# LeeBY68/Hier-SLAM

Measured on AMD Instinct MI355X. Metric: fwd+bwd renders/sec @1200x680, 500k Gaussians, 4-level tree; grad max-abs-err vs ref, higher is better.
Workload: dtype f32; 1 GPU; semantic fwd+bwd render, 1200x680, P=500000 slam Gaussians, K=26 semantic channels, dense upstream grads on colour/semantic/depth/median/opacity; P=500000, visible=480888, num_rendered=1136056, width=1200, height=680, K=26, parallelism=single GPU, keyframes_per_rank=1

## Files before the change

### hier-slam_amd/csrc/hsr_render_bwd_q.hip

```cpp
#include "hsr_bwd_tile.h"

#ifdef HSR_TRACE
#define HSR_TRACE_SLOTS 8
__device__ unsigned long long g_hsr_trace_q[16384 * HSR_TRACE_SLOTS];
extern "C" int hsr_debug_read_trace_q(unsigned long long* host, int n)
{
    return (int)hipMemcpyFromSymbol(host, HIP_SYMBOL(g_hsr_trace_q), sizeof(unsigned long long) * (size_t)n);
}
#define TR_NOW() clock64()
#define TR_ADD(acc, t0) (acc) += (unsigned long long)(clock64() - (t0))
#else
#define TR_NOW() 0ll
#define TR_ADD(acc, t0) ((void)0)
#endif

namespace {

constexpr int Q_ROWS = 16;
constexpr int Q_CAP = 40;
constexpr int Q_SEG_DUMMY = Q_CAP;
constexpr int Q_SEG_ZERO = Q_CAP + 1;
constexpr int Q_NSEG = Q_CAP + 2;
constexpr int Q_SEGW = 17;
constexpr int Q_SEGB = Q_SEGW * 4;
constexpr int Q_PANEL = Q_NSEG * Q_SEGW;
constexpr int Q_ORD = 20;
constexpr int Q_TB = 36;
constexpr int Q_ENTB = 48;
static_assert(2 * Q_PANEL >= 64 * 17, "the two panels double as the prologue's transposition scratch");
static_assert(Q_ROWS * Q_TB <= Q_SEG_ZERO * Q_SEGW, "the emission table overlays the W panel below its zero segment");

template <int KC, int BATCH, bool GEO, bool CL = false, bool SEMA = false>
__global__ void __launch_bounds__(256, (SEMA || (!GEO && KC + 5 > 16)) ? 3 : 4) render_bwd_q_kernel(RenderBwdArgs a)
{
    static_assert(!SEMA || (GEO && KC % 4 == 0 && KC > 0), "the semantic -> alpha pass is a geometry-only pass over whole float4s of features");
    constexpr int ENTB = SEMA ? Q_ENTB + 4 * KC : Q_ENTB;
    constexpr int REC4 = ENTB / 16;
    constexpr int NCH = GEO ? 0 : KC + 5;
    constexpr int NG = GEO ? 0 : (NCH + 15) / 16;
    constexpr int NGA = NG > 0 ? NG : 1;
    static_assert(NG <= 2, "at most 32 direct channels per launch");
    static_assert(BATCH <= 256 && (BATCH + 1) * ENTB < 65536, "batch slots are bytes, record offsets 16 bits");
    __shared__ float4 s_ent[REC4 * (BATCH + 1)];
    __shared__ int s_id[BATCH];
    __shared__ uint16_t s_mask[BATCH + 2];
    __shared__ uint8_t s_list[4][256];
    __shared__ uint8_t s_lcnt[4][4];
    __shared__ uint8_t s_flat[4][256];
    __shared__ int s_wmax[4];
    __shared__ __attribute__((aligned(16))) float s_pan[4][2 * Q_PANEL];
    __shared__ uint2 s_ord[4][4][Q_ORD];
    __shared__ uint32_t s_rowent[4][Q_ROWS];
    __shared__ __attribute__((aligned(16))) uint32_t s_cid[4][Q_ROWS];
    __shared__ float s_medj[BATCH];
    __shared__ uint8_t s_segtab[4][Q_ROWS][4];

    const int tile = hsr_block_tile(blockIdx.x, hsr_num_tiles(a.W, a.H));
    if (tile >= hsr_num_tiles(a.W, a.H)) return;
    const int t = threadIdx.x, lane = t & 63, wv = t >> 6, gq = lane >> 4, l16 = lane & 15;
    const TileGeom tg = tile_geom_sub(tile, a.W, a.H, t);
    const bool inside = tg.inside;
    const size_t N = (size_t)a.W * a.H;
    const size_t pix_id = (size_t)a.W * tg.py + tg.px;
    float pfx = tg.pfx, pfy = tg.pfy;
    asm volatile("" : "+v"(pfx), "+v"(pfy));
    const uint2 range = a.ranges[tile];
    float* pw = s_pan[wv];
    float* pq = s_pan[wv] + Q_PANEL;
    unsigned long long tr_stage = 0, tr_loop = 0, tr_flush = 0, tr_iters = 0, tr_chunks = 0, tr_accepted = 0, tr_setup = 0;
    (void)tr_setup;
    const long long tr_t0 = TR_NOW();
    (void)tr_stage; (void)tr_loop; (void)tr_flush; (void)tr_iters; (void)tr_chunks; (void)tr_accepted; (void)tr_t0;

    if (t < REC4) s_ent[REC4 * BATCH + t] = make_float4(0.f, 0.f, 0.f, 0.f);

    const size_t pix_ld = inside ? pix_id : 0;
    const float inm = inside ? 1.f : 0.f;
    const float T_final_ld = a.final_T[pix_ld];
    const int last_contributor_ld = (int)a.n_contrib[pix_ld];
    const int median_at_ld = (int)a.median_pos[pix_ld];
    float dpx0 = a.dL_dpix[pix_ld], dpx1 = a.dL_dpix[N + pix_ld], dpx2 = a.dL_dpix[2 * N + pix_ld];
    float dpd = a.dL_dpix_depth[pix_ld], dpm = a.dL_dpix_median[pix_ld], dpo = a.dL_dpix_opacity[pix_ld];
    float semv[KC > 0 ? KC : 1];
#pragma unroll
    for (int c = 0; c < KC; c++) semv[c] = a.dL_dpix_sem[(size_t)min((SEMA ? a.sem_c0 : 0) + c, a.K - 1) * N + pix_ld];
    if (SEMA) {
#pragma unroll
        for (int c = 0; c < KC; c++) semv[c] = (a.sem_c0 + c < a.K) ? semv[c] * inm : 0.f;
        dpx0 = dpx1 = dpx2 = dpd = dpm = dpo = 0.f;
    }
    dpx0 *= inm; dpx1 *= inm; dpx2 *= inm; dpd *= inm; dpm *= inm; dpo *= inm;
    const float T_final = T_final_ld * inm;
    float T = T_final;
    const int last_contributor = inside ? last_contributor_ld : 0;
    const int median_at = (inside ? median_at_ld : 0) - 1;

    int wmax = last_contributor;
#pragma unroll
    for (int o = 32; o > 0; o >>= 1) wmax = max(wmax, __shfl_xor(wmax, o));
    if (lane == 0) s_wmax[wv] = wmax;

    float Breg[NGA][16];
    if (!GEO) {
        float gv[NGA][16];
#pragma unroll
        for (int g = 0; g < NG; g++)
#pragma unroll
            for (int c = 0; c < 16; c++) {
                const int ch = 16 * g + c;
                float v = 0.f;
                if (ch < KC) {
                    v = (ch < a.K) ? semv[ch < KC ? ch : 0] * inm : 0.f;
                } else if (ch == KC) v = dpx0;
                else if (ch == KC + 1) v = dpx1;
                else if (ch == KC + 2) v = dpx2;
                else if (ch == KC + 3) v = dpd;
                else if (ch == KC + 4) v = dpo;
                gv[g][c] = v;
            }
#pragma unroll
        for (int g = 0; g < NG; g++) {
            HSR_BWD_TRANSPOSE_B(pw, lane, gv[g], Breg[g]);
        }
    }
    if (lane < 2 * Q_SEGW) {
        if (GEO) pw[Q_SEG_ZERO * 2 * Q_SEGW + lane] = 0.f;
        else (lane < Q_SEGW ? pw : pq - Q_SEGW)[Q_SEG_ZERO * Q_SEGW + lane] = 0.f;
    }
    __syncthreads();
    const int hi_all = max(max(s_wmax[0], s_wmax[1]), max(s_wmax[2], s_wmax[3]));
    const long long tr_t1 = TR_NOW();
    (void)tr_t1;

    const float ntfbg = -T_final * (a.bg[0] * dpx0 + a.bg[1] * dpx1 + a.bg[2] * dpx2);
    const float kx2 = (a.W) / HSR_LOG2E, ky2 = (a.H) / HSR_LOG2E;
    float Racc = 0.f;
    char* const panb = reinterpret_cast<char*>(&s_pan[0][0]);
    const char* const entb = reinterpret_cast<const char*>(&s_ent[0]);
    constexpr uint32_t SEGB = GEO ? 2 * Q_SEGB : Q_SEGB;
    const uint32_t wave_off = (uint32_t)(wv * 2 * Q_PANEL * 4);
    const uint32_t lane16_off = wave_off + (uint32_t)(l16 * (GEO ? 8 : 4));
    const uint2 DUMMY_ELEM = make_uint2((uint32_t)(BATCH * ENTB), (uint32_t)Q_SEG_DUMMY * SEGB);
    uint2* const ordp = &s_ord[wv][gq][0];

    HSR_BWD_STAGING_DECLARE();
    HSR_BWD_STAGING_PRIME(hi_all, BATCH);

    auto flush = [&](int nrows) {
        wave_lds_fence();
        const uint32_t st = *reinterpret_cast<const uint32_t*>(&s_segtab[wv][l16][0]);
        const float cxg = pfx - (float)(l16 & 3) + 1.5f, cyg = pfy - (float)(l16 >> 2) + 1.5f;
        constexpr bool ALL_IN_LINE0 = CL && NCH <= 9;
        int colg[NGA], tslot[NGA];
#pragma unroll
        for (int g = 0; g < NGA; g++) {
            const int ch = 16 * g + l16;
            const int chl = ch < KC ? (ch < a.K ? ch : -1) : (ch < KC + 5 ? a.K + (ch - KC) : -1);
            const int col = (GEO || chl < 0) ? -1 : hsr_grow_col(CL ? 1 : 0, a.K, chl);
            colg[g] = (col >= 16 && !ALL_IN_LINE0) ? col : -1;
            tslot[g] = (CL && col >= 7 && col < 16) ? col - 7 : -1;
        }
        f32x4 acc[NGA];
#pragma unroll
        for (int g = 0; g < NGA; g++) acc[g] = f32x4{0.f, 0.f, 0.f, 0.f};
        if (!GEO) {
            float av[16];
#pragma unroll
            for (int g4 = 0; g4 < 4; g4++) {
                const float* sp = pw + ((st >> (8 * g4)) & 0xFFu) * Q_SEGW + gq;
#pragma unroll
                for (int i = 0; i < 4; i++) av[4 * g4 + i] = sp[4 * i];
            }
            asm volatile("" : "+v"(av[0]), "+v"(av[1]), "+v"(av[2]), "+v"(av[3]), "+v"(av[4]), "+v"(av[5]), "+v"(av[6]), "+v"(av[7]));
            asm volatile("" : "+v"(av[8]), "+v"(av[9]), "+v"(av[10]), "+v"(av[11]), "+v"(av[12]), "+v"(av[13]), "+v"(av[14]), "+v"(av[15]));
            if (NG == 1) {
                f32x4 acc2 = f32x4{0.f, 0.f, 0.f, 0.f};
#pragma unroll
                for (int m = 0; m < 16; m += 2) {
                    acc[0] = __builtin_amdgcn_mfma_f32_16x16x4f32(av[m], Breg[0][m], acc[0], 0, 0, 0);
                    acc2 = __builtin_amdgcn_mfma_f32_16x16x4f32(av[m + 1], Breg[0][m + 1], acc2, 0, 0, 0);
                }
                acc[0] += acc2;
            } else {
#pragma unroll
                for (int m = 0; m < 16; m++)
#pragma unroll
                    for (int g = 0; g < NG; g++)
                        acc[g] = __builtin_amdgcn_mfma_f32_16x16x4f32(av[m], Breg[g][m], acc[g], 0, 0, 0);
            }
        }
        float o[7];
        const uint32_t myseg = (st >> (8 * gq)) & 0xFFu;
        float qv[16], wd[GEO ? 16 : 1], medsum;
        if (GEO) {
            const float2* qp = reinterpret_cast<const float2*>(pw) + myseg * Q_SEGW;
#pragma unroll
            for (int i = 0; i < 16; i++) {
                const float2 v = qp[i];
                qv[i] = v.x;
                wd[GEO ? i : 0] = v.y;
            }
            medsum = 0.f;
        } else {
            const float* qp = pq + myseg * Q_SEGW;
#pragma unroll
            for (int i = 0; i < 16; i++) qv[i] = qp[i];
            medsum = 0.f;
        }
        const uint32_t eo = s_rowent[wv][l16];
        if (!SEMA && gq == 0 && eo < (uint32_t)(BATCH * ENTB)) medsum = atomicExch(&s_medj[eo / ENTB], 0.f);
        const float4* ent = reinterpret_cast<const float4*>(entb + eo);
        const float4 e0 = ent[0], e2 = ent[2];
        float s0[4], s1[4], s2[4];
#pragma unroll
        for (int yy = 0; yy < 4; yy++) {
            const float qa = qv[4 * yy], qb = qv[4 * yy + 1], qc = qv[4 * yy + 2], qd = qv[4 * yy + 3];
            const float ad = qa + qd, bc = qb + qc;
            s0[yy] = ad + bc;
            s1[yy] = fmaf(1.5f, qd - qa, 0.5f * (qc - qb));
            s2[yy] = fmaf(2.25f, ad, 0.25f * bc);
        }
        const float M0 = (s0[0] + s0[3]) + (s0[1] + s0[2]);
        const float Mu = (s1[0] + s1[3]) + (s1[1] + s1[2]);
        const float Muu = (s2[0] + s2[3]) + (s2[1] + s2[2]);
        const float Mv = fmaf(1.5f, s0[3] - s0[0], 0.5f * (s0[2] - s0[1]));
        const float Mvv = fmaf(2.25f, s0[0] + s0[3], 0.25f * (s0[1] + s0[2]));
        const float Muv = fmaf(1.5f, s1[3] - s1[0], 0.5f * (s1[2] - s1[1]));
        const float ex = e0.x - cxg, ey = e0.y - cyg;
        const float Ap = e0.z, Cp = e2.x, op = e2.y, hB = e2.z;
        const float Sx = fmaf(fmaf(Ap, ex, hB * ey), M0, -fmaf(Ap, Mu, hB * Mv));
        const float Sy = fmaf(fmaf(Cp, ey, hB * ex), M0, -fmaf(Cp, Mv, hB * Mu));
        const float Sxx = fmaf(ex, fmaf(ex, M0, -2.0f * Mu), Muu);
        const float Sxy = fmaf(ex, fmaf(ey, M0, -Mv), fmaf(-ey, Mu, Muv));
        const float Syy = fmaf(ey, fmaf(ey, M0, -2.0f * Mv), Mvv);
        const float mh = -0.5f * op;
        o[0] = (kx2 * op) * Sx;
        o[1] = (ky2 * op) * Sy;
        o[2] = mh * Sxx;
        o[3] = mh * Sxy;
        o[4] = mh * Syy;
        o[5] = M0;
        float s6 = medsum;
        if (GEO) {
            float wsum[4];
#pragma unroll
            for (int yy = 0; yy < 4; yy++) wsum[yy] = (wd[GEO ? 4 * yy : 0] + wd[GEO ? 4 * yy + 1 : 0]) + (wd[GEO ? 4 * yy + 2 : 0] + wd[GEO ? 4 * yy + 3 : 0]);
            s6 += (wsum[0] + wsum[1]) + (wsum[2] + wsum[3]);
        }
        o[6] = s6;
        if (!GEO && !ALL_IN_LINE0) {
            const uint4 b4 = *reinterpret_cast<const uint4*>(&s_cid[wv][4 * (lane >> 4)]);
            const uint32_t bb[4] = {b4.x, b4.y, b4.z, b4.w};
            const int nr = nrows - 4 * (lane >> 4);
#pragma unroll
            for (int r = 0; r < 4; r++)
#pragma unroll
                for (int g = 0; g < NG; g++)
                    if (r < nr && colg[g] >= 0)
                        atomicAdd(reinterpret_cast<float*>(reinterpret_cast<char*>(a.grow) + 4u * (bb[r] + (uint32_t)colg[g])), acc[g][r]);
        }
        if (CL && !GEO) {
            wave_lds_fence();
#pragma unroll
            for (int g = 0; g < NG; g++)
                if (tslot[g] >= 0) {
#pragma unroll
                    for (int r = 0; r < 4; r++) pq[(4 * (lane >> 4) + r) * 12 + tslot[g]] = acc[g][r];
                }
        }
        wave_lds_fence();
        float* tb = pw;
#pragma unroll
        for (int vi = 0; vi < 7; vi++) tb[l16 * Q_TB + 4 * vi + gq] = o[vi];
        wave_lds_fence();
        if (CL && !GEO) {
            const int nl0 = hsr_grow_nl0(a.K);
            const int vi = lane & 15;
            float4 sa[4];
            float ta[4];
            uint32_t cid[4];
#pragma unroll
            for (int pass = 0; pass < 4; pass++) {
                const int row = (lane >> 4) + 4 * pass;
                sa[pass] = *reinterpret_cast<const float4*>(tb + row * Q_TB + (vi & 7) * 4);
                ta[pass] = pq[row * 12 + min(max(vi - 7, 0), 11)];
                cid[pass] = s_cid[wv][row];
            }
            asm volatile("" : "+v"(sa[0].x), "+v"(sa[1].x), "+v"(sa[2].x), "+v"(sa[3].x), "+v"(ta[0]), "+v"(ta[1]), "+v"(ta[2]), "+v"(ta[3]),
                         "+v"(cid[0]), "+v"(cid[1]), "+v"(cid[2]), "+v"(cid[3]));
#pragma unroll
            for (int pass = 0; pass < 4; pass++) {
                const int row = (lane >> 4) + 4 * pass;
                const float val = vi < 7 ? (sa[pass].x + sa[pass].y) + (sa[pass].z + sa[pass].w) : ta[pass];
                if (vi < 7 + nl0 && row < nrows && val != 0.f)
                    atomicAdd(reinterpret_cast<float*>(reinterpret_cast<char*>(a.grow) + 4u * (cid[pass] + (uint32_t)vi)), val);
            }
        } else {
            const int vi = lane & 7;
            float4 sa[2];
            uint32_t cid[2];
#pragma unroll
            for (int pass = 0; pass < 2; pass++) {
                const int row = (lane >> 3) + 8 * pass;
                sa[pass] = *reinterpret_cast<const float4*>(tb + row * Q_TB + vi * 4);
                cid[pass] = s_cid[wv][row];
            }
            asm volatile("" : "+v"(sa[0].x), "+v"(sa[1].x), "+v"(cid[0]), "+v"(cid[1]));
#pragma unroll
            for (int pass = 0; pass < 2; pass++) {
                const int row = (lane >> 3) + 8 * pass;
                const float val = (sa[pass].x + sa[pass].y) + (sa[pass].z + sa[pass].w);
                if (vi < 7 && row < nrows && val != 0.f)
                    atomicAdd(reinterpret_cast<float*>(reinterpret_cast<char*>(a.grow) + 4u * (cid[pass] + (uint32_t)vi)), val);
            }
        }
        wave_lds_fence();
    };

    for (int hi = hi_all; hi > 0; hi -= BATCH) {
        const int cnt = min(BATCH, hi);
        const int jf_off = (hi - last_contributor) * ENTB;
        const long long ts = TR_NOW();
        (void)ts;
        __syncthreads();
        uint32_t qmask = 0u;
        if (t < cnt) {
            const uint32_t mask = p_mask;
            qmask = quadrant_bits(mask);
            s_mask[t] = (uint16_t)mask;
            s_id[t] = id_cur;
            s_medj[t] = 0.f;
            HSR_BWD_STORE_RECORD(s_ent, REC4 * t);
            if (SEMA) {
                const float* f = a.semantics + (size_t)id_cur * (size_t)a.K;
#pragma unroll
                for (int q = 0; q < KC / 4; q++) {
                    float v[4];
#pragma unroll
                    for (int i = 0; i < 4; i++) {
                        const int ch = a.sem_c0 + 4 * q + i;
                        v[i] = ch < a.K ? f[ch] : 0.f;
                    }
                    s_ent[REC4 * t + 3 + q] = make_float4(v[0], v[1], v[2], v[3]);
                }
            }
        }
        publish_quadrant_lists(qmask, t, s_list, s_lcnt);
        __syncthreads();
        {
            const int jm = hi - 1 - median_at;
            if (jm >= 0 && jm < cnt && dpm != 0.f) atomicAdd(&s_medj[jm], dpm);
        }
        HSR_BWD_STAGING_ADVANCE(hi, BATCH);
        TR_ADD(tr_stage, ts);
        if (hi - cnt >= wmax) {
            HSR_SETTLE_STAGING();
            continue;
        }
        const long long tl = TR_NOW();
        (void)tl;

        const int total = build_flat_list(wv, lane, s_list, s_lcnt, s_flat);
        if (total == 0) HSR_SETTLE_STAGING();
        int nrows = 0;
        for (int c0 = 0; c0 < total; c0 += nrows) {
            nrows = min(Q_ROWS, total - c0);
            const long long tsu = TR_NOW();
            (void)tsu;
            const int jr = l16 < nrows ? (int)s_flat[wv][c0 + l16] : BATCH;
            bool touch = l16 < nrows && ((s_mask[jr] >> (4 * wv + gq)) & 1u);
            uint64_t ball = __ballot(touch);
            if (__popcll(ball) > Q_CAP) {
                nrows = Q_CAP / 4;
                touch = touch && l16 < nrows;
                ball = __ballot(touch);
            }
            const uint32_t eoff = (uint32_t)(l16 < nrows ? jr : BATCH) * (uint32_t)ENTB;
            if (gq == 0) {
                s_rowent[wv][l16] = eoff;
                s_cid[wv][l16] = (uint32_t)s_id[min(jr, BATCH - 1)] * (uint32_t)a.grow_stride;
            }
            const uint32_t seg = touch ? __builtin_amdgcn_mbcnt_hi((uint32_t)(ball >> 32), __builtin_amdgcn_mbcnt_lo((uint32_t)ball, 0u)) : (uint32_t)Q_SEG_ZERO;
            s_segtab[wv][l16][gq] = (uint8_t)seg;
            ordp[l16] = DUMMY_ELEM;
            if (l16 < Q_ORD - 16) ordp[16 + l16] = DUMMY_ELEM;
            const uint32_t gmask = (uint32_t)(ball >> (16 * gq)) & 0xFFFFu;
            if (touch) {
                ordp[__popc(gmask & ((1u << l16) - 1u))] = make_uint2(eoff, seg * SEGB);
            }
            const int iters = longest_group_list(ball);
            wave_lds_fence();
            struct StageA { float am, Gm, inv, nb, h; uint32_t ro; };
            auto stage_a = [&](const float4& ra, const float4& rb, const float2& rc, uint2 e) -> StageA {
                StageA o;
                const int eo = (int)e.x;
                o.ro = lane16_off + e.y;
                const float dx = ra.x - pfx, dy = ra.y - pfy;
                const float dxx = dx * dx, dxy = dx * dy, dyy = dy * dy;
                const float power2 = fmaf(rc.x, dyy, fmaf(ra.w, dxy, ra.z * dxx));
                const float G = __builtin_amdgcn_exp2f(power2);
                const float alpha = fminf(0.99f, rc.y * G);
                const bool active = eo >= jf_off && power2 <= 0.0f && alpha >= 1.0f / 255.0f;
#ifdef HSR_TRACE
                {
                    const uint64_t ba = __ballot(active);
#pragma unroll
                    for (int gg = 0; gg < 4; gg++) tr_accepted += ((ba >> (16 * gg)) & 0xFFFFull) != 0ull;
                    tr_iters += 1;
                }
#endif
                o.am = active ? alpha : 0.f;
                o.Gm = active ? G : 0.f;
                o.inv = __builtin_amdgcn_rcpf(1.0f - o.am);
                o.nb = ntfbg * o.inv;
                if (SEMA) {
                    const float4* f = reinterpret_cast<const float4*>(entb + e.x + Q_ENTB);
                    float h0 = 0.f, h1 = 0.f;
#pragma unroll
                    for (int q = 0; q < KC / 4; q++) {
                        const float4 v = f[q];
                        h0 = fmaf(v.x, semv[SEMA ? 4 * q : 0], fmaf(v.y, semv[SEMA ? 4 * q + 1 : 0], h0));
                        h1 = fmaf(v.z, semv[SEMA ? 4 * q + 2 : 0], fmaf(v.w, semv[SEMA ? 4 * q + 3 : 0], h1));
                    }
                    o.h = h0 + h1;
                } else {
                    o.h = fmaf(rb.x, dpx0, fmaf(rb.y, dpx1, fmaf(rb.z, dpx2, fmaf(rb.w, dpd, dpo))));
                }
                return o;
            };
            auto stage_b = [&](const StageA& c) {
                const float test_T = T * c.inv;
                const float w = c.am * test_T;
                const float d = c.h - Racc;
                const float dL_dalpha = fmaf(d, test_T, c.nb);
                const float gda = c.Gm * dL_dalpha;
                if (GEO) {
                    *reinterpret_cast<float2*>(panb + c.ro) = make_float2(gda, w * dpd);
                } else {
                    *reinterpret_cast<float*>(panb + c.ro) = w;
                    *reinterpret_cast<float*>(panb + c.ro + Q_PANEL * 4) = gda;
                }
                Racc = fmaf(c.am, d, Racc);
                T = test_T;
            };
            auto load_rec = [&](uint2 e, float4& ra, float4& rb, float2& rc) {
                const float4* ent = reinterpret_cast<const float4*>(entb + e.x);
                ra = ent[0];
                rb = ent[1];
                rc = *reinterpret_cast<const float2*>(&ent[2]);
            };
            uint2 e1 = ordp[1], e2 = ordp[2];
            float4 ra1, rb1;
            float2 rc1;
            StageA cur;
            {
                const uint2 e0 = ordp[0];
                float4 ra0, rb0;
                float2 rc0;
                load_rec(e0, ra0, rb0, rc0);
                load_rec(e1, ra1, rb1, rc1);
                cur = stage_a(ra0, rb0, rc0, e0);
            }
#ifdef HSR_TRACE
            asm volatile("" ::"v"(cur.am), "v"(cur.h), "v"(ra1.x), "v"(rb1.x));
#endif
            TR_ADD(tr_setup, tsu);
            for (int it = 0; it < iters; it += 2) {
                const uint2 e3 = ordp[it + 3];
                float4 ra2, rb2;
                float2 rc2;
                load_rec(e2, ra2, rb2, rc2);
                const StageA nxt = stage_a(ra1, rb1, rc1, e1);
                stage_b(cur);
                const uint2 e4 = ordp[it + 4];
                load_rec(e3, ra1, rb1, rc1);
                cur = stage_a(ra2, rb2, rc2, e2);
                stage_b(nxt);
                e1 = e3; e2 = e4;
            }
            {
                const long long tf = TR_NOW();
                (void)tf;
                if (c0 == 0) HSR_SETTLE_STAGING();
                flush(nrows);
                TR_ADD(tr_flush, tf);
#ifdef HSR_TRACE
                tr_chunks++;
#endif
            }
        }
        TR_ADD(tr_loop, tl);
    }
#ifdef HSR_TRACE
    if (lane == 0) {
        const int wid = tile * 4 + wv;
        if (wid < 16384) {
            unsigned long long* o = g_hsr_trace_q + (size_t)wid * HSR_TRACE_SLOTS;
            o[0] = (unsigned long long)(clock64() - tr_t0);
            o[1] = (unsigned long long)(tr_t1 - tr_t0);
            o[2] = tr_stage; o[3] = tr_loop; o[4] = tr_flush; o[5] = tr_chunks; o[6] = tr_iters; o[7] = tr_setup;
        }
    }
#endif
}

}

int hsr_launch_render_backward_q(const RenderBwdArgs& a, hipStream_t stream)
{
    const dim3 grid(hsr_tile_grid(hsr_num_tiles(a.W, a.H))), block(256);
    const int K = a.semantic ? a.K : 0;
    const bool cl = a.grow_layout == 1;
    if (K < 0 || K > 27 || (K == 0 && !cl) || !a.grow || a.grow_stride != hsr_grow_stride_l(a.grow_layout, K) ||
        !hsr_rows_fit_32bit(a.P, a.grow_stride)) {
        hsr_set_error("Q-panel backward kernel: needs 0 <= K <= 27 (got %d; compact rows at K = 0), packed rows of the layout's stride (got %d) and P * stride < 2^30", K, a.grow_stride);
        return HSR_ERR_INVALID_ARGUMENT;
    }
    if (K == 0) render_bwd_q_kernel<0, 208, false, true><<<grid, block, 0, stream>>>(a);
    else if (K <= 11) {
        if (cl) render_bwd_q_kernel<11, 208, false, true><<<grid, block, 0, stream>>>(a);
        else render_bwd_q_kernel<11, 208, false, false><<<grid, block, 0, stream>>>(a);
    } else if (K == 16 && cl) render_bwd_q_kernel<16, 224, false, true><<<grid, block, 0, stream>>>(a);
    else if (K == 26 && !cl) render_bwd_q_kernel<26, 224, false, false><<<grid, block, 0, stream>>>(a);
    else if (cl) render_bwd_q_kernel<27, 224, false, true><<<grid, block, 0, stream>>>(a);
    else render_bwd_q_kernel<27, 224, false, false><<<grid, block, 0, stream>>>(a);
    return HSR_OK;
}

int hsr_launch_render_backward_qsema(const RenderBwdArgs& a0, hipStream_t stream)
{
    RenderBwdArgs a = a0;
    const dim3 grid(hsr_tile_grid(hsr_num_tiles(a.W, a.H))), block(256);
    for (int c0 = 0; c0 < a.K; c0 += 16) {
        a.sem_c0 = c0;
        render_bwd_q_kernel<16, 208, true, false, true><<<grid, block, 0, stream>>>(a);
    }
    return HSR_OK;
}

int hsr_launch_render_backward_qgeo(const RenderBwdArgs& a, hipStream_t stream)
{
    if (!a.grow || a.grow_stride != 16 || !hsr_rows_fit_32bit(a.P, 16)) {
        hsr_set_error("geometry-only backward kernel: needs packed rows of 16 floats (got stride %d) and P * 16 < 2^30", a.grow_stride);
        return HSR_ERR_INVALID_ARGUMENT;
    }
    render_bwd_q_kernel<0, 208, true><<<dim3(hsr_tile_grid(hsr_num_tiles(a.W, a.H))), dim3(256), 0, stream>>>(a);
    return HSR_OK;
}
```

Before: 1751 renders/s.

## Merge per-Gaussian line-0 gradient atomics in LDS before global emission

For two-group channel launches without CL, the per-row line-0 gradient contributions (7 values, including the median-depth term) are now accumulated into a per-batch LDS table via shared atomics. Each batch's table is flushed to global memory once, at the next batch boundary and after the loop, instead of each wave chunk issuing its own global atomics. The median-depth sum moves into slot 6 of that table, replacing the atomicExch path. This cuts global atomic traffic and contention. In exchange it adds LDS usage (BATCH*32 bytes, which may affect occupancy), extra shared atomics, and a flush pass at each batch boundary.

```diff
diff --git a/hier-slam_amd/csrc/hsr_render_bwd_q.hip b/hier-slam_amd/csrc/hsr_render_bwd_q.hip
--- a/hier-slam_amd/csrc/hsr_render_bwd_q.hip
+++ b/hier-slam_amd/csrc/hsr_render_bwd_q.hip
@@ -39,6 +39,7 @@
     constexpr int NCH = GEO ? 0 : KC + 5;
     constexpr int NG = GEO ? 0 : (NCH + 15) / 16;
     constexpr int NGA = NG > 0 ? NG : 1;
+    constexpr bool MERGE = NG == 2 && !CL;
     static_assert(NG <= 2, "at most 32 direct channels per launch");
     static_assert(BATCH <= 256 && (BATCH + 1) * ENTB < 65536, "batch slots are bytes, record offsets 16 bits");
     __shared__ float4 s_ent[REC4 * (BATCH + 1)];
@@ -52,7 +53,8 @@
     __shared__ uint2 s_ord[4][4][Q_ORD];
     __shared__ uint32_t s_rowent[4][Q_ROWS];
     __shared__ __attribute__((aligned(16))) uint32_t s_cid[4][Q_ROWS];
-    __shared__ float s_medj[BATCH];
+    __shared__ float s_medj[MERGE ? 1 : BATCH];
+    __shared__ __attribute__((aligned(16))) float s_l0[MERGE ? BATCH : 1][8];
     __shared__ uint8_t s_segtab[4][Q_ROWS][4];
 
     const int tile = hsr_block_tile(blockIdx.x, hsr_num_tiles(a.W, a.H));
@@ -208,7 +210,7 @@
             medsum = 0.f;
         }
         const uint32_t eo = s_rowent[wv][l16];
-        if (!SEMA && gq == 0 && eo < (uint32_t)(BATCH * ENTB)) medsum = atomicExch(&s_medj[eo / ENTB], 0.f);
+        if (!SEMA && !MERGE && gq == 0 && eo < (uint32_t)(BATCH * ENTB)) medsum = atomicExch(&s_medj[eo / ENTB], 0.f);
         const float4* ent = reinterpret_cast<const float4*>(entb + eo);
         const float4 e0 = ent[0], e2 = ent[2];
         float s0[4], s1[4], s2[4];
@@ -303,18 +305,44 @@
             for (int pass = 0; pass < 2; pass++) {
                 const int row = (lane >> 3) + 8 * pass;
                 sa[pass] = *reinterpret_cast<const float4*>(tb + row * Q_TB + vi * 4);
-                cid[pass] = s_cid[wv][row];
+                cid[pass] = MERGE ? s_rowent[wv][row] : s_cid[wv][row];
             }
             asm volatile("" : "+v"(sa[0].x), "+v"(sa[1].x), "+v"(cid[0]), "+v"(cid[1]));
 #pragma unroll
             for (int pass = 0; pass < 2; pass++) {
                 const int row = (lane >> 3) + 8 * pass;
                 const float val = (sa[pass].x + sa[pass].y) + (sa[pass].z + sa[pass].w);
-                if (vi < 7 && row < nrows && val != 0.f)
-                    atomicAdd(reinterpret_cast<float*>(reinterpret_cast<char*>(a.grow) + 4u * (cid[pass] + (uint32_t)vi)), val);
+                if (vi < 7 && row < nrows && val != 0.f) {
+                    if (MERGE) atomicAdd(&s_l0[MERGE ? cid[pass] / (uint32_t)ENTB : 0u][vi], val);
+                    else atomicAdd(reinterpret_cast<float*>(reinterpret_cast<char*>(a.grow) + 4u * (cid[pass] + (uint32_t)vi)), val);
+                }
             }
         }
         wave_lds_fence();
+    };
+
+    auto emit_line0 = [&](int n) {
+        int tt = t;
+        asm volatile("" : "+v"(tt));
+        const int vi = tt & 7, slot0 = (tt & ~63) + ((tt & 63) >> 3);
+#pragma unroll
+        for (int half = 0; half < 2; half++) {
+            float val[4];
+            uint32_t rid[4];
+#pragma unroll
+            for (int pass = 0; pass < 4; pass++) {
+                const int slot = min(slot0 + 32 * half + 8 * pass, BATCH - 1);
+                val[pass] = s_l0[MERGE ? slot : 0][vi];
+                rid[pass] = (uint32_t)s_id[slot] * (uint32_t)a.grow_stride;
+            }
+            asm volatile("" : "+v"(val[0]), "+v"(val[1]), "+v"(val[2]), "+v"(val[3]), "+v"(rid[0]), "+v"(rid[1]), "+v"(rid[2]), "+v"(rid[3]));
+#pragma unroll
+            for (int pass = 0; pass < 4; pass++) {
+                const int slot = slot0 + 32 * half + 8 * pass;
+                if (slot < n && vi < 7 && val[pass] != 0.f)
+                    atomicAdd(reinterpret_cast<float*>(reinterpret_cast<char*>(a.grow) + 4u * (rid[pass] + (uint32_t)vi)), val[pass]);
+            }
+        }
     };
 
     for (int hi = hi_all; hi > 0; hi -= BATCH) {
@@ -323,13 +351,17 @@
         const long long ts = TR_NOW();
         (void)ts;
         __syncthreads();
+        if (MERGE && hi != hi_all) emit_line0(BATCH);
         uint32_t qmask = 0u;
         if (t < cnt) {
             const uint32_t mask = p_mask;
             qmask = quadrant_bits(mask);
             s_mask[t] = (uint16_t)mask;
             s_id[t] = id_cur;
-            s_medj[t] = 0.f;
+            if (MERGE) {
+                *reinterpret_cast<float4*>(&s_l0[MERGE ? t : 0][0]) = make_float4(0.f, 0.f, 0.f, 0.f);
+                *reinterpret_cast<float4*>(&s_l0[MERGE ? t : 0][4]) = make_float4(0.f, 0.f, 0.f, 0.f);
+            } else s_medj[t] = 0.f;
             HSR_BWD_STORE_RECORD(s_ent, REC4 * t);
             if (SEMA) {
                 const float* f = a.semantics + (size_t)id_cur * (size_t)a.K;
@@ -349,7 +381,7 @@
         __syncthreads();
         {
             const int jm = hi - 1 - median_at;
-            if (jm >= 0 && jm < cnt && dpm != 0.f) atomicAdd(&s_medj[jm], dpm);
+            if (jm >= 0 && jm < cnt && dpm != 0.f) atomicAdd(MERGE ? &s_l0[MERGE ? jm : 0][6] : &s_medj[MERGE ? 0 : jm], dpm);
         }
         HSR_BWD_STAGING_ADVANCE(hi, BATCH);
         TR_ADD(tr_stage, ts);
@@ -491,6 +523,10 @@
         }
         TR_ADD(tr_loop, tl);
     }
+    if (MERGE && hi_all > 0) {
+        __syncthreads();
+        emit_line0((hi_all - 1) % BATCH + 1);
+    }
 #ifdef HSR_TRACE
     if (lane == 0) {
         const int wid = tile * 4 + wv;
```

Measured after the change: 1798 renders/s, median of 6. +2.7%, better.
